# DeepLearnPhysics/u-resnet

Measured on AMD Instinct MI355X. Metric: fwd+bwd images/sec on 3D 192^3x1 U-ResNet, higher is better.
Workload: dtype f32; 1 GPU; cfg3_3d192_f8_b4; base_filters=8, num_class=3, batch_per_gpu=4, global_batch=4, step=zero_gradients+accum_gradients(fwd+loss+bwd)+allreduce+adam, parallelism=dp1

## Files before the change

### u-resnet_amd/csrc/conv_api.hip

```cpp
#include <dlfcn.h>
#include <stdarg.h>
#include <stdlib.h>
#include <stdio.h>
#include <string.h>

#include "bf16_common.h"

static thread_local char g_err[1024] = "";
void ursn_set_error(const char* fmt, ...) {
  va_list ap;
  va_start(ap, fmt);
  vsnprintf(g_err, sizeof(g_err), fmt, ap);
  va_end(ap);
}
extern "C" const char* ursn_last_error(void) { return g_err; }
static thread_local const char* g_kernel = "";
static long g_kernel_launches = 0;
void ursn_note_kernel(const char* name) { g_kernel = name; ++g_kernel_launches; }
void ursn_relabel_kernel(const char* name) { g_kernel = name; }
long ursn_kernel_launch_count() { return g_kernel_launches; }
extern "C" const char* ursn_last_kernel_name() { return g_kernel; }
extern "C" int ursn_abi_version(void) { return URSN_ABI_VERSION; }

namespace {
// ... 208 lines not shown
    if (g[i].ntaps == 0 && accumulate) continue;
    if (d.algo == 1) URSN_TRY(launch_gconv_naive(g[i], in, w, out, s));
    else URSN_TRY(launch_gconv_mfma(g[i], in, w, out, s));
  }
  return 0;
}

int tiled_conv_supported(const ursn_conv_desc& d, ConvPass pass);
int launch_tiled_conv(const ursn_conv_desc& d, ConvPass pass, const float* in, const float* w, float* out,
                      int accumulate, hipStream_t s);

static float* op_scratch_floats(size_t n) {
  static float* buf = nullptr;
  static size_t cap = 0;
  if (n > cap) {
    if (buf) (void)hipFree(buf);
    buf = nullptr; cap = 0;
    if (hipMalloc((void**)&buf, n * sizeof(float)) != hipSuccess) return nullptr;
    cap = n;
  }
  return buf;
}

int conv_dispatch(const ursn_conv_desc& d, ConvPass pass, const float* in, const float* w, float* out, int accumulate,
                  hipStream_t s) {
  if (d.vdz_z) {
    URSN_REQUIRE(pass == PASS_DGRAD && d.vdz_coef && d.vdz_out && tiled_conv_supported(d, pass), "conv: BatchNorm-backward apply on load (vdz_z) not supported for this shape / pass");
    return launch_tiled_conv(d, pass, in, w, out, accumulate, s);
  }
  if (d.bs_partial) {
    URSN_REQUIRE(pass == PASS_DGRAD && tiled_conv_supported(d, pass), "conv: fused BatchNorm-backward reductions (bs_partial) not supported for this shape / pass");
    return launch_tiled_conv(d, pass, in, w, out, accumulate, s);
  }
  if (d.in_mean && pass != PASS_DGRAD) {
    URSN_REQUIRE(d.in_rstd && d.in_beta && tiled_conv_supported(d, pass), "conv: normalise-on-load (in_mean) not supported for this shape / pass");
    return launch_tiled_conv(d, pass, in, w, out, accumulate, s);
  }
  if (d.pw_dy) {
    URSN_REQUIRE(pass == PASS_DGRAD, "conv: fused pointwise term (pw_dy) applies to the data gradient only");
    if (tiled_deconv_supported(d, pass))
      return launch_tiled_deconv(d, pass, in, w, out, accumulate, nullptr, 0.f, nullptr, nullptr, s);
    if (!d.in_split && igemm_conv_supported(d, pass))
      return launch_igemm_conv(d, pass, in, w, out, accumulate, nullptr, 0.f, nullptr, nullptr, s);
    URSN_REQUIRE(tiled_conv_supported(d, pass), "conv: fused pointwise term (pw_dy) not supported for this shape");
    return launch_tiled_conv(d, pass, in, w, out, accumulate, s);
  }
  if (d.in_split) {
    if (pointwise_conv_supported(d, pass, accumulate))
      return launch_pointwise_conv(d, pass, in, w, out, accumulate, nullptr, 0.f, nullptr, nullptr, s);
    URSN_REQUIRE(tiled_conv_supported(d, pass), "conv: split input (in_split=%d) not supported for this shape", d.in_split);
    return launch_tiled_conv(d, pass, in, w, out, accumulate, s);
  }
  if (d.algo == 3) {
    if (tiled_deconv_supported(d, pass))
// ... 215 lines not shown
    return launch_tiled_conv_bn(*d, x, w, y, (double*)scratch, eps, mean, rstd, s);
  }
  URSN_REQUIRE(reduce_scratch_bytes(V, d->cout, 2) <= scratch_bytes, "conv_forward_stats: scratch too small");
  URSN_TRY(conv_dispatch(*d, PASS_FWD, x, w, y, 0, s));
  return launch_bn_stats(y, ocs, V, d->cout, eps, mean, rstd, scratch, s);
}

extern "C" int ursn_conv_backward_data(const ursn_conv_desc* d, const float* dy, const float* w, float* dx,
                                       int32_t accumulate, void* stream) {
  URSN_REQUIRE(d && dy && w && dx, "conv_backward_data: null argument");
  if (d->dtype == 1) return bf16_conv_op(*d, PASS_DGRAD, dy, w, dx, accumulate, nullptr, 0, 0.f, nullptr, nullptr, (hipStream_t)stream);
  return conv_dispatch(*d, PASS_DGRAD, dy, w, dx, accumulate, (hipStream_t)stream);
}

int tiled_wgrad_supported(const ursn_conv_desc& d);
size_t tiled_wgrad_scratch_bytes(const ursn_conv_desc& d);
int valu_wgrad_supported(const ursn_conv_desc& d);
size_t valu_wgrad_scratch_bytes(const ursn_conv_desc& d);
int launch_valu_wgrad(const ursn_conv_desc& d, const float* x, const float* dy, float* dw, void* scratch, size_t scratch_bytes,
                      hipStream_t s);
int launch_tiled_wgrad(const ursn_conv_desc& d, const float* x, const float* dy, float* dw, void* scratch,
                       size_t scratch_bytes, hipStream_t s);

extern "C" int32_t ursn_conv_bs_blocks(const ursn_conv_desc* d) { return d ? tiled_conv_bs_blocks(*d) : 0; }

extern "C" int ursn_conv_plan(const ursn_conv_desc* d0, int32_t pass_, char* out, size_t cap) {
  URSN_REQUIRE(d0 && out && cap > 0 && pass_ >= 0 && pass_ <= 2, "conv_plan: bad argument");
  const ConvPass pass = (ConvPass)pass_;
  ursn_conv_desc d = *d0;
  const char* name = "gather";
  GatherGeom g[8];
  if (d.dtype == 1) {
    if (d.cin == 1) { d.cin = 8; d.in_cstride = 8; }
    const int n = build_geoms(d, pass, g);
    URSN_REQUIRE(n >= 1, "conv_plan: bad descriptor");
    int first = 0;
    while (first < n - 1 && g[first].ntaps == 0) ++first;
    if (pass == PASS_WGRAD) name = (d0->cin == 1 && b0wgrad_ok(g[0])) ? "b0wgrad" : b3wgrad_ok(g[0]) ? "b3wgrad" : bdwgrad_ok(g[0]) ? "bdwgrad" : bs2k8w_ok(g[0]) ? "bs2k8w" : (bwgrad_scratch_bytes(g[0]) ? "bwgrad" : "none");
    else if (d0->cin == 1 && pass == PASS_FWD && n == 1 && b0conv_ok(g[0])) name = "b0conv";
    else if (n == 1 && bs2k8_ok(g[0])) name = "bs2k8";
    else if (bdeconv_ok(g, n)) name = "bdeconv";
    else if (bsconv_ok(g, n)) name = "bsconv";
    else if (bpw_ok(g[first])) name = "bpw";
    else if (b3conv_ok(g[first])) name = "b3conv";
    else if (bcbconv_ok(g[first])) name = "bcbconv";
    else if (bdconv_ok(g[first])) name = "bdconv";
    else name = bconv_pack_elems(g[first]) ? "bconv" : "none";
    snprintf(out, cap, "%s", name);
    return 0;
  }
  URSN_REQUIRE(build_geoms(d, pass, g) >= 1, "conv_plan: bad descriptor");
  if (pass == PASS_WGRAD) {
    if (d.in_mean || (d.in_split && !pointwise_wgrad_supported(d))) name = tiled_wgrad_supported(d) ? "twgrad" : "none";
    else if (pointwise_wgrad_supported(d)) name = "pwgrad";
    else if (deep_wgrad_supported(d)) name = "dwgrad";
    else if (igemm_wgrad_supported(d)) name = "igemm_wgrad";
    else if (valu_wgrad_supported(d)) name = "vwgrad";
    else if (tiled_wgrad_supported(d)) name = "twgrad";
    else if (stride2_wgrad_supported(d)) name = "s2wgrad";
    else name = "wgrad_mfma";
  } else {
    if (d.vdz_z || d.bs_partial || (d.in_mean && pass != PASS_DGRAD)) name = tiled_conv_supported(d, pass) ? "tconv" : "none";
    else if (d.pw_dy && tiled_deconv_supported(d, pass)) name = "tdeconv+pw";
    else if (d.pw_dy) name = (!d.in_split && igemm_conv_supported(d, pass)) ? "igemm" : (tiled_conv_supported(d, pass) ? "tconv" : "none");
    else if (d.in_split) name = pointwise_conv_supported(d, pass, 0) ? "pconv" : (tiled_conv_supported(d, pass) ? "tconv" : "none");
    else if (pointwise_conv_supported(d, pass, 0)) name = "pconv";
    else if (deep_conv_supported(d, pass)) name = "dconv";
    else if (igemm_conv_supported(d, pass)) name = "igemm";
    else if (tiled_conv_supported(d, pass)) name = "tconv";
    else if (prefer_lds_scatter(d, pass)) name = "s2scatter";
    else if (tiled_deconv_supported(d, pass)) name = "tdeconv";
    else if (stride2_conv_supported(d, pass)) name = "s2conv";
    else name = "gconv_mfma";
  }
  snprintf(out, cap, "%s", name);
  return 0;
}

extern "C" size_t ursn_conv_wgrad_scratch_bytes(const ursn_conv_desc* d) {
  if (!d) return 0;
  GatherGeom g[8];
  if (d->dtype == 1) {
    ursn_conv_desc dd = *d;
    if (dd.cin == 1) { dd.cin = 8; dd.in_cstride = 8; }
    if (build_geoms(dd, PASS_WGRAD, g) != 1) return 0;
// ... 200 lines not shown
```

### u-resnet_amd/csrc/conv_igemm.hip

```cpp
#include <stdlib.h>

#include "conv_igemm_kernel.h"

bool ursn_igemm_on() {
  static const bool v = ursn_env_on("URSN_IGEMM");
  return v;
}

static bool make_igplan(const ursn_conv_desc& d, ConvPass pass, IGPlan& p, int& kcin, int& kcout) {
  if ((ursn_tiled_disabled() || !ursn_igemm_on()) && d.algo != 4) return false;
  if (d.transposed || d.k != 3 || d.stride != 1 || d.in_split || d.in_mean) return false;
  if (pass != PASS_FWD && pass != PASS_DGRAD) return false;
  p.flip = (pass == PASS_DGRAD);
  kcin = p.flip ? d.cout : d.cin;
  kcout = p.flip ? d.cin : d.cout;
  if ((kcin % 16) || (kcout % 16)) return false;
  if (kcin <= 16 && kcout <= 16 && d.algo != 4) return false;
  const int ics = d.in_cstride > 0 ? d.in_cstride : d.cin, ocs = d.out_cstride > 0 ? d.out_cstride : d.cout;
  if ((ics & 3) || (ocs & 3)) return false;
  p.mode = d.ndim;
  if (d.ndim == 3) { p.Z = d.in_sp[0]; p.Y = d.in_sp[1]; p.X = d.in_sp[2]; }
  else { p.Z = 1; p.Y = d.in_sp[0]; p.X = d.in_sp[1]; }
  static const int min_x = ursn_env_int("URSN_IGEMM_MINX", 5);
  if (p.X < min_x && d.algo != 4) return false;
  static const int at = ursn_env_int("URSN_IGEMM_ALLTAPS", 1);
  p.var = 0;
  if (at && p.mode == 3 && p.X <= 12) p.var = (p.X <= 6) ? 2 : 1;
  const bool at32 = at >= 1 && at != 16;
  if (!p.var && at32 && p.mode == 3 && (p.X % 16) != 0 && (p.X % 16) <= 8 && (p.X % 12) == 0) p.var = 1;
  if (p.X < 12 && !p.var && d.algo != 4) return false;
  const int BZ = p.mode == 3 ? (p.var == 2 ? 3 : 4) : 1, BY = p.mode == 3 ? (p.var == 2 ? 6 : 4) : 16,
            BX = p.var == 2 ? 6 : (p.var == 1 ? 12 : 16);
  p.nbz = (p.Z + BZ - 1) / BZ;
  p.nby = (p.Y + BY - 1) / BY;
  p.nbx = (p.X + BX - 1) / BX;
  p.gridx = d.n * p.nbz * p.nby * p.nbx;
  if (p.var == 2 || (p.var == 1 && !(at32 && kcout >= 32 && (int64_t)p.gridx * (kcout / 32) >= 384))) p.bm = 16;
  else if (p.var == 1) p.bm = 32;
  else if (kcout >= 64 && p.gridx >= 512) p.bm = 64;
  else if (kcout >= 32 && (int64_t)p.gridx * (kcout / 32) >= 384) p.bm = 32;
  else p.bm = 16;
  p.gridy = (kcout + p.bm - 1) / p.bm;
  const int HZ = p.mode == 3 ? BZ + 2 : 1, HY = BY + 2, HX = BX + 2;
  p.lds = ((size_t)4 * HZ * HY * HX * 4 + (size_t)2 * 16 * (p.bm + 16)) * sizeof(float);
  p.alltaps = (at && p.bm == 16) || (at >= 1 && at != 16 && p.bm == 32);
  if (d.pw_dy && !(p.flip && p.alltaps)) return false;
  if (p.alltaps) {
    {
      const int ics = d.in_cstride > 0 ? d.in_cstride : d.cin, ocs = d.out_cstride > 0 ? d.out_cstride : d.cout;
      if ((int64_t)p.Z * p.Y * p.X * (p.flip ? ocs : ics) * 4 >= (int64_t)0x80000000ll) return false;
    }
    const int kc = p.bm == 16 ? 16 : 8;
    p.lds = ((size_t)(kc / 4) * HZ * HY * HX * 4 + (size_t)(p.mode == 3 ? 27 : 9) * kc * p.bm) * sizeof(float);
    if (d.pw_dy) {
      const int nv = BZ * BY * BX;
      p.lds += ((size_t)(kc / 4) * nv * 4 + (size_t)p.bm * kc) * sizeof(float);
    }
    static const int pad_kb = ursn_env_int("URSN_IGEMM_LDS_KB", 0);
    if (pad_kb > 0 && p.lds < (size_t)pad_kb * 1024) p.lds = (size_t)pad_kb * 1024;
  }
  return true;
}

int igemm_conv_supported(const ursn_conv_desc& d, ConvPass pass) {
  IGPlan p;
  int a, b;
  return make_igplan(d, pass, p, a, b) ? 1 : 0;
}

size_t igemm_stats_scratch_doubles(const ursn_conv_desc& d) {
  IGPlan p;
  int a, b;
  if (!make_igplan(d, PASS_FWD, p, a, b)) return 0;
  return (size_t)p.gridx * p.gridy * 2 * p.bm;
}

template <int MODE, int BM>
static int dispatch_flags(const IGPlan& p, const IGemmArgs& a, hipStream_t s) {
  if (p.flip) return launch_ig<MODE, BM, true, false>(p, a, s);
  if (a.stats_partial) return launch_ig<MODE, BM, false, true>(p, a, s);
  return launch_ig<MODE, BM, false, false>(p, a, s);
}

template <int MODE>
static int dispatch_bm(const IGPlan& p, const IGemmArgs& a, hipStream_t s) {
  if (p.bm == 64) { ursn_note_kernel(p.flip ? "igemm_dgrad<64>" : "igemm<64>"); return dispatch_flags<MODE, 64>(p, a, s); }
  if (p.bm == 32 && p.alltaps) {
    ursn_note_kernel(p.flip ? "igemm_at_dgrad<32>" : "igemm_at<32>");
    if constexpr (MODE == 3) {
      if (p.var == 1) {
        if (p.flip) return launch_ig_at<3, 32, 8, true, false, 1>(p, a, s);
        if (a.stats_partial) return launch_ig_at<3, 32, 8, false, true, 1>(p, a, s);
        return launch_ig_at<3, 32, 8, false, false, 1>(p, a, s);
      }
    }
    if (p.flip) return launch_ig_at<MODE, 32, 8, true, false>(p, a, s);
    if (a.stats_partial) return launch_ig_at<MODE, 32, 8, false, true>(p, a, s);
    return launch_ig_at<MODE, 32, 8, false, false>(p, a, s);
  }
  if (p.bm == 32) { ursn_note_kernel(p.flip ? "igemm_dgrad<32>" : "igemm<32>"); return dispatch_flags<MODE, 32>(p, a, s); }
  if (p.alltaps) {
    ursn_note_kernel(p.flip ? "igemm_at_dgrad<16>" : "igemm_at<16>");
    if constexpr (MODE == 3) {
      if (p.var == 1) {
        if (p.flip) return launch_ig_at<3, 16, 16, true, false, 1>(p, a, s);
        if (a.stats_partial) return launch_ig_at<3, 16, 16, false, true, 1>(p, a, s);
        return launch_ig_at<3, 16, 16, false, false, 1>(p, a, s);
      }
      if (p.var == 2) {
        if (p.flip) return launch_ig_at<3, 16, 16, true, false, 2>(p, a, s);
        if (a.stats_partial) return launch_ig_at<3, 16, 16, false, true, 2>(p, a, s);
        return launch_ig_at<3, 16, 16, false, false, 2>(p, a, s);
      }
    }
    if (p.flip) return launch_ig_at<MODE, 16, 16, true, false>(p, a, s);
    if (a.stats_partial) return launch_ig_at<MODE, 16, 16, false, true>(p, a, s);
    return launch_ig_at<MODE, 16, 16, false, false>(p, a, s);
  }
  ursn_note_kernel(p.flip ? "igemm_dgrad<16>" : "igemm<16>");
  return dispatch_flags<MODE, 16>(p, a, s);
}

int launch_igemm_conv(const ursn_conv_desc& d, ConvPass pass, const float* in, const float* w, float* out,
                      int accumulate, double* stats_partial, float eps, float* mean, float* rstd, hipStream_t s) {
  IGPlan p;
  int kcin, kcout;
  URSN_REQUIRE(make_igplan(d, pass, p, kcin, kcout), "igemm conv: unsupported shape");
  const int ics = d.in_cstride > 0 ? d.in_cstride : d.cin, ocs = d.out_cstride > 0 ? d.out_cstride : d.cout;
  IGemmArgs a;
  a.in = in; a.w = w; a.out = out; a.stats_partial = stats_partial;
  a.N = d.n; a.Z = p.Z; a.Y = p.Y; a.X = p.X;
  a.cin = kcin; a.cout = kcout;
  a.in_cs = p.flip ? ocs : ics;
  a.out_cs = p.flip ? ics : ocs;
  a.cin_w = d.cin; a.cout_w = d.cout;
  a.nbz = p.nbz; a.nby = p.nby; a.nbx = p.nbx;
  a.accumulate = accumulate;
  a.pw_in = nullptr; a.pw_w = nullptr; a.pw_cs = 0; a.pw_ws = 0;
  if (d.pw_dy) {
    URSN_REQUIRE(p.flip && p.alltaps && d.pw_w, "igemm conv: fused pointwise term needs the all-taps data-gradient kernel");
    a.pw_in = d.pw_dy; a.pw_w = d.pw_w;
    a.pw_cs = d.pw_dy_cstride > 0 ? d.pw_dy_cstride : d.cout;
    a.pw_ws = d.cout;
    URSN_REQUIRE((a.pw_cs & 3) == 0, "igemm conv: pw_dy channel stride must be a multiple of 4");
  }
  URSN_TRY(p.mode == 3 ? dispatch_bm<3>(p, a, s) : dispatch_bm<2>(p, a, s));
  if (stats_partial) {
    const int64_t V = (int64_t)d.n * p.Z * p.Y * p.X;
    URSN_TRY(launch_bn_stats_final_blocked(stats_partial, p.gridx, kcout, p.bm, p.bm, (size_t)p.gridx * 2 * p.bm, V, eps, mean, rstd, s));
  }
  return 0;
}
```

### u-resnet_amd/csrc/conv_igemm_kernel.h

```cpp
#pragma once
#include <utility>

#include "ursn_common.h"
#include "buffer_stage.h"

typedef float ig_f32x4 __attribute__((ext_vector_type(4)));

template <int... Is, class F>
__device__ __forceinline__ void ig_static_for_impl(std::integer_sequence<int, Is...>, F&& f) {
  (f(std::integral_constant<int, Is>{}), ...);
}
template <int N, class F>
__device__ __forceinline__ void ig_static_for(F&& f) {
  ig_static_for_impl(std::make_integer_sequence<int, N>{}, static_cast<F&&>(f));
}

struct IGemmArgs {
  const float* in;
  const float* w;
  float* out;
  double* stats_partial;
  int N, Z, Y, X;
  int cin, cout;
  int in_cs, out_cs;
  int cin_w, cout_w;
  int nbz, nby, nbx;
  int accumulate;
  const float* pw_in;
  const float* pw_w;
  int pw_cs, pw_ws;
};

template <int MODE> struct IBox;
template <> struct IBox<3> { static constexpr int BZ = 4, BY = 4, BX = 16, NT = 27, KZ = 3; };
template <> struct IBox<2> { static constexpr int BZ = 1, BY = 16, BX = 16, NT = 9, KZ = 1; };
template <int MODE, int VAR> struct ABox : IBox<MODE> {};
template <> struct ABox<3, 1> { static constexpr int BZ = 4, BY = 4, BX = 12, NT = 27, KZ = 3; };
template <> struct ABox<3, 2> { static constexpr int BZ = 3, BY = 6, BX = 6, NT = 27, KZ = 3; };

template <int MODE, int BM, bool FLIP, bool STATS>
__global__ __launch_bounds__(256, 2) void igemm_conv_kernel(IGemmArgs a) {
  using B = IBox<MODE>;
  constexpr int BZ = B::BZ, BY = B::BY, BX = B::BX, NT = B::NT, KZ = B::KZ;
  constexpr int HZ = BZ + (KZ - 1), HY = BY + 2, HX = BX + 2, PS = HZ * HY * HX;
  constexpr int KC = 16, WS = BM + 16;
  constexpr int MT = BM / 16;
  constexpr int NH = (4 * PS + 255) / 256;
  extern __shared__ __attribute__((aligned(16))) float ilds[];
  float* hal = ilds;
  float* wl = ilds + 4 * PS * 4;

  const int tid = threadIdx.x, lane = tid & 63, wave = tid >> 6;
  const int il = lane & 15, kl = lane >> 4;
// ... 119 lines not shown
  }
  if constexpr (STATS) if (a.stats_partial) {
    __shared__ double red[4][2 * BM];
#pragma unroll
    for (int m = 0; m < MT; ++m)
#pragma unroll
      for (int r = 0; r < 4; ++r) {
        double u, w2;
        ursn_sacc_final(piv[m][r], s1[m][r], s2[m][r], nacc[m], u, w2);
#pragma unroll
        for (int o = 8; o >= 1; o >>= 1) { u += __shfl_xor(u, o); w2 += __shfl_xor(w2, o); }
        if (il == 0) {
          red[wave][16 * m + 4 * kl + r] = u;
          red[wave][BM + 16 * m + 4 * kl + r] = w2;
        }
      }
    __syncthreads();
    if (tid < 2 * BM)
      a.stats_partial[((size_t)blockIdx.y * gridDim.x + blockIdx.x) * 2 * BM + tid] =
          (red[0][tid] + red[1][tid]) + (red[2][tid] + red[3][tid]);
  }
}

template <int MODE, int BM, int KC, bool FLIP, bool STATS, int VAR = 0>
__global__ __launch_bounds__(256, 2) void igemm_at_kernel(IGemmArgs a) {
  using B = ABox<MODE, VAR>;
  constexpr int BZ = B::BZ, BY = B::BY, BX = B::BX, NT = B::NT, KZ = B::KZ;
  constexpr int NV = BZ * BY * BX, TPW = (NV + 63) / 64;
  constexpr int HZ = BZ + (KZ - 1), HY = BY + 2, HX = BX + 2, PS = HZ * HY * HX;
  constexpr int MT = BM / 16, NQ = KC / 4;
  constexpr int NH = (NQ * PS + 255) / 256;
  constexpr int NWF = NT * KC * BM / 4;
  constexpr int NW = (NWF + 255) / 256;
  extern __shared__ __attribute__((aligned(16))) float ilds[];
  float* hal = ilds;
  float* wl = ilds + NQ * PS * 4;

  const int tid = threadIdx.x, lane = tid & 63, wave = tid >> 6;
  const int il = lane & 15, kl = lane >> 4;
  int bid = ursn_xcd_block(blockIdx.x, gridDim.x);
  const int bx = bid % a.nbx; bid /= a.nbx;
  const int by = bid % a.nby; bid /= a.nby;
  const int bz = bid % a.nbz;
  const int n = bid / a.nbz;
  const int x0 = bx * BX, y0 = by * BY, z0 = bz * BZ;
  const int co0 = blockIdx.y * BM;

// ... 159 lines not shown
    if (pw) {
#pragma unroll
      for (int s = 0; s < NQ; ++s) {
        float av[MT], bv[TPW];
#pragma unroll
        for (int m = 0; m < MT; ++m) av[m] = pww[wb + ((size_t)m * KC + 4 * s) * 16];
#pragma unroll
        for (int v = 0; v < TPW; ++v) bv[v] = pwx[((size_t)s * NV + (vox[v] < 0 ? 0 : vox[v])) * 4 + kl];
#pragma unroll
        for (int v = 0; v < TPW; ++v)
#pragma unroll
          for (int m = 0; m < MT; ++m) acc[v][m] = __builtin_amdgcn_mfma_f32_16x16x4f32(av[m], bv[v], acc[v][m], 0, 0, 0);
      }
    }
  }

  float s1[MT][4], s2[MT][4], piv[MT][4], nacc[MT];
#pragma unroll
  for (int m = 0; m < MT; ++m) {
    nacc[m] = 0.f;
#pragma unroll
    for (int r = 0; r < 4; ++r) s1[m][r] = s2[m][r] = piv[m][r] = 0.f;
  }
#pragma unroll
  for (int v = 0; v < TPW; ++v) {
    if (vox[v] < 0) continue;
    const int lx = vox[v] % BX, r = vox[v] / BX;
    const int gx = x0 + lx, gy = y0 + r % BY, gz = z0 + r / BY;
    if (!(gz < a.Z && gy < a.Y && gx < a.X)) continue;
    float* op = a.out + ((((size_t)n * a.Z + gz) * a.Y + gy) * a.X + gx) * a.out_cs + co0;
#pragma unroll
    for (int m = 0; m < MT; ++m) {
      const int c = 16 * m + 4 * kl;
      if (co0 + c >= a.cout) continue;
      ig_f32x4 val = acc[v][m];
      if (a.accumulate) val += *(ig_f32x4*)(op + c);
      *(ig_f32x4*)(op + c) = val;
      if constexpr (STATS) {
#pragma unroll
        for (int r = 0; r < 4; ++r) {
          if (nacc[m] == 0.f) piv[m][r] = val[r];
          ursn_sacc(piv[m][r], s1[m][r], s2[m][r], val[r]);
        }
        nacc[m] += 1.f;
      }
    }
  }
  if constexpr (STATS) if (a.stats_partial) {
    __shared__ double red[4][2 * BM];
#pragma unroll
    for (int m = 0; m < MT; ++m)
#pragma unroll
      for (int r = 0; r < 4; ++r) {
        double u, w2;
        ursn_sacc_final(piv[m][r], s1[m][r], s2[m][r], nacc[m], u, w2);
#pragma unroll
        for (int o = 8; o >= 1; o >>= 1) { u += __shfl_xor(u, o); w2 += __shfl_xor(w2, o); }
        if (il == 0) {
          red[wave][16 * m + 4 * kl + r] = u;
          red[wave][BM + 16 * m + 4 * kl + r] = w2;
        }
      }
    __syncthreads();
    if (tid < 2 * BM)
      a.stats_partial[((size_t)blockIdx.y * gridDim.x + blockIdx.x) * 2 * BM + tid] =
          (red[0][tid] + red[1][tid]) + (red[2][tid] + red[3][tid]);
  }
}

struct IGPlan {
  bool alltaps;
  int var;
  int mode, bm;
  bool flip;
  int Z, Y, X, nbz, nby, nbx;
  size_t lds;
  int gridx, gridy;
};

template <int MODE, int BM, int KC, bool FLIP, bool STATS, int VAR = 0>
static int launch_ig_at(const IGPlan& p, const IGemmArgs& a, hipStream_t s) {
  auto kern = igemm_at_kernel<MODE, BM, KC, FLIP, STATS, VAR>;
  static size_t attr_lds = 48 * 1024;
  if (p.lds > attr_lds) {
    URSN_HIP(hipFuncSetAttribute((const void*)kern, hipFuncAttributeMaxDynamicSharedMemorySize, (int)p.lds));
    attr_lds = p.lds;
  }
  hipLaunchKernelGGL(kern, dim3(p.gridx, p.gridy), dim3(256), p.lds, s, a);
  URSN_HIP(hipGetLastError());
  return 0;
}

template <int MODE, int BM, bool FLIP, bool STATS>
static int launch_ig(const IGPlan& p, const IGemmArgs& a, hipStream_t s) {
  auto kern = igemm_conv_kernel<MODE, BM, FLIP, STATS>;
  static size_t attr_lds = 48 * 1024;
  if (p.lds > attr_lds) {
    URSN_HIP(hipFuncSetAttribute((const void*)kern, hipFuncAttributeMaxDynamicSharedMemorySize, (int)p.lds));
    attr_lds = p.lds;
  }
  hipLaunchKernelGGL(kern, dim3(p.gridx, p.gridy), dim3(256), p.lds, s, a);
  URSN_HIP(hipGetLastError());
  return 0;
}
```

### u-resnet_amd/csrc/net.hip

```cpp
#include <math.h>
#include <stdio.h>
#include <stdlib.h>
#include <string.h>

#include <map>
#include <string>
#include <vector>

#include "ursn_common.h"
#include "net_bf16.h"

int conv_dispatch(const ursn_conv_desc& d, ConvPass pass, const float* in, const float* w, float* out, int accumulate,
                  hipStream_t s);
int wgrad_dispatch(const ursn_conv_desc& d, const float* x, const float* dy, float* dw, void* scratch,
                   size_t scratch_bytes, hipStream_t s);

namespace {

struct Act {
  float* p = nullptr;
  float* g = nullptr;
  int C = 0, cs = 0, lvl = 0;
  int flag = -1;
};

struct Layer {
  std::string name;
  int kind = 0;
  int k = 3, stride = 1, cin = 0, cout = 0, lin = 0, lout = 0;
  int relu = 0;
  int64_t w_off = 0, b_off = 0, w_n = 0;
  ursn_conv_desc desc;
  float *z = nullptr, *dz = nullptr, *mean = nullptr, *rstd = nullptr;
  float* coef = nullptr;
  int zcs = 0;
};

struct Unit {
  std::string scope;
  int sc = -1, c1 = -1, c2 = -1;
// ... 284 lines not shown
      }
    }
  }
  n->red_scratch = A.take(red + 256);
  n->dc_scratch = dcf ? A.floats((int64_t)dcf + 64) : nullptr;
  {
    size_t red2 = 0;
    for (const Unit& u : n->units) {
      if (u.sc < 0) continue;
      const Layer& L = n->layers[u.sc];
      size_t r = reduce_scratch_bytes((int64_t)c.max_batch * n->lvox[L.lout], L.cout, 3);
      if (r > red2) red2 = r;
      for (int nb = 1; nb <= c.max_batch; ++nb) {
        ursn_conv_desc d = L.desc;
        d.n = nb;
        r = pointwise_stats_scratch_doubles(d) * sizeof(double);
        if (r > red2) red2 = r;
      }
    }
    n->red_scratch2 = A.take(red2 + 256);
  }
  n->wg_scratch_bytes = wg;
  n->wg_scratch = tr ? A.take(wg + 256) : nullptr;
  n->bs_scratch = tr ? (double*)A.take((size_t)16384 * 3 * 8 * sizeof(double)) : nullptr;

  n->sizes.n_params = poff;
  n->sizes.n_layers = (int64_t)n->layers.size();
  n->sizes.n_tensors = 2 * (int64_t)n->layers.size();
  n->sizes.workspace_bytes = (int64_t)((A.off + 255) & ~(size_t)255);
  return 0;
}

extern "C" const char* ursn_last_kernel_name();
hipEvent_t prof_event(ursn_net* n) {
  if (n->ev_used == n->ev_pool.size()) {
    hipEvent_t e;
    if (hipEventCreate(&e) != hipSuccess) return nullptr;
    n->ev_pool.push_back(e);
  }
  return n->ev_pool[n->ev_used++];
}
struct ProfScope {
  ursn_net* n; hipStream_t s; int idx = -1; bool range = false;
  ProfScope(ursn_net* n_, hipStream_t s_, int layer, int pass, double flops, double bytes) : n(n_), s(s_) {
    if (ursn_roctx_on()) { ursn_roctx_push(n->layers[layer].name.c_str(), pass); range = true; }
    if (!n->profile || n->prof.size() > 200000) return;
    ursn_net::ProfRec r{layer, pass, "", flops, bytes, prof_event(n), prof_event(n), ursn_kernel_launch_count(), 1};
    if (!r.e0 || !r.e1) return;
    hipEventRecord(r.e0, s);
    n->prof.push_back(r);
    idx = (int)n->prof.size() - 1;
  }
  ~ProfScope() { if (range) ursn_roctx_pop(); }
  void done(const char* kernel) {
    if (idx < 0) return;
    n->prof[idx].kernel = kernel;
    long nl = ursn_kernel_launch_count() - n->prof[idx].l0;
    n->prof[idx].launches = nl > 0 ? (int)nl : 1;
    hipEventRecord(n->prof[idx].e1, s);
  }
};
double layer_macs(const ursn_net* n, const Layer& L, int N) {
  double taps = 1;
  for (int j = 0; j < n->cfg.ndim; ++j) taps *= L.k;
  double vox = (double)N * (L.kind ? n->lvox[L.lin] : n->lvox[L.lout]);
  return vox * taps * L.cin * L.cout;
}
double layer_bytes(const ursn_net* n, const Layer& L, int N) {
  return 4.0 * ((double)N * n->lvox[L.lin] * L.cin + (double)N * n->lvox[L.lout] * L.cout + (double)L.w_n);
}

int conv_stats(ursn_net* n, int li, const Act& in, int N, hipStream_t s, const Act* in2 = nullptr, int aff = -1,
               void* red_scratch = nullptr) {
  if (!red_scratch) red_scratch = n->red_scratch;
  Layer& L = n->layers[li];
  ursn_conv_desc d = L.desc;
  d.n = N;
  d.in_cstride = in.cs;
  d.out_cstride = L.zcs;
  if (in2) { d.in_split = in.C; d.in2_cstride = in2->cs; d.x2 = in2->p; }
  if (aff >= 0) {
// ... 253 lines not shown
    URSN_TRY(wgrad_dispatch(d, in.p, L.dz, n->grads + L.w_off, n->wg_scratch, n->wg_scratch_bytes, ws));
    ps.done(ursn_last_kernel_name());
  }
  if (dgrad_done_elsewhere) {
    ProfScope pd(n, s, li, 1, 2.0 * layer_macs(n, L, N), layer_bytes(n, L, N));
    pd.done("(fused into conv1 dgrad)");
  }
  if (need_dgrad) {
    bool acc = take_flag(n, in);
    if (in2) URSN_REQUIRE(take_flag(n, *in2) == acc, "split input: the two halves disagree on gradient initialisation");
    d = bwd_desc(n, li, in, N, in2, fused_sc);
    n->bs_layer = -1;
    static const bool bs_off = !ursn_env_on("URSN_FUSE_BN_BWD_REDUCE");
    if (bs && bs->li >= 0 && !bs_off) {
      const Layer& T = n->layers[bs->li];
      ursn_conv_desc t = d;
      t.bs_z = T.z; t.bs_z_cstride = T.zcs; t.bs_mean = T.mean; t.bs_rstd = T.rstd; t.bs_beta = n->params + T.b_off;
      t.bs_relu = bs->relu; t.bs_mask = bs->mask;
      if (bs->li2 >= 0) {
        const Layer& T2 = n->layers[bs->li2];
        t.bs_z2 = T2.z; t.bs_z2_cstride = T2.zcs; t.bs_mean2 = T2.mean; t.bs_rstd2 = T2.rstd;
      }
      t.bs_partial = n->bs_scratch;
      const bool fits = T.cout == 8 && T.zcs == 8 && in.C == 8 && in.cs == 8 && !in2 &&
                        (bs->li2 < 0 || n->layers[bs->li2].zcs == 8) && (bs->relu != 2 || bs->mask);
      const int blocks = fits ? tiled_conv_bs_blocks(t) : 0;
      if (blocks > 0 && blocks <= 16384) { d = t; n->bs_layer = bs->li; n->bs_blocks = blocks; }
    }
    ProfScope pd(n, s, li, 1, 2.0 * layer_macs(n, L, N), layer_bytes(n, L, N));
    if (n->dc_scratch && deep_conv_supported(d, PASS_DGRAD))
      URSN_TRY(launch_deep_conv(d, PASS_DGRAD, L.dz, n->params + L.w_off, in.g, acc ? 1 : 0, n->dc_scratch, nullptr, 0.f, nullptr, nullptr, s));
    else
      URSN_TRY(conv_dispatch(d, PASS_DGRAD, L.dz, n->params + L.w_off, in.g, acc ? 1 : 0, s));
    pd.done(ursn_last_kernel_name());
  }
  return 0;
}

bool vdz_ok(ursn_net* n, int li, const Act& in, int N, bool two_z_target) {
  static const bool on = ursn_env_on("URSN_FUSE_BN_BWD_APPLY");
  const bool off = !on || two_z_target;
  const Layer& L = n->layers[li];
  if (off || n->cfg.ndim != 3 || L.kind || L.k != 3 || L.stride != 1 || L.cin != 8 || L.cout != 8 || L.zcs != 8 || in.C != 8 || in.cs != 8 || !in.g)
    return false;
  ursn_conv_desc d = L.desc;
  d.n = N; d.in_cstride = in.cs; d.out_cstride = L.zcs;
  d.vdz_z = L.z; d.vdz_coef = L.coef; d.vdz_out = L.dz;
  return tiled_conv_supported(d, PASS_DGRAD) != 0;
}

// ... 3 lines not shown
  Layer& L = n->layers[li];
  BnBwdArgs a;
  memset(&a, 0, sizeof(a));
  a.dy = dy; a.dycs = dycs; a.y = mask ? nullptr : y; a.ycs = ycs; a.mask = mask;
  a.z = L.z; a.zcs = L.zcs; a.mean = L.mean; a.rstd = L.rstd; a.dz = L.dz; a.dzcs = L.zcs;
  a.dbeta = n->grads + L.b_off;
  a.beta = n->params + L.b_off;
  if (li2 >= 0) {
    Layer& L2 = n->layers[li2];
    a.z2 = L2.z; a.z2cs = L2.zcs; a.mean2 = L2.mean; a.rstd2 = L2.rstd; a.dz2 = L2.dz; a.dz2cs = L2.zcs;
    a.dbeta2 = n->grads + L2.b_off;
  }
  a.dres = dres; a.drescs = drescs; a.dres_accumulate = dres_acc;
  a.V = (int64_t)N * n->lvox[L.lout]; a.C = L.cout; a.relu = relu; a.scratch = n->red_scratch;
  if (L.zcs != L.cout && li2 < 0 && !relu && dycs == L.zcs && !dres) { a.C = L.zcs; a.Cw = L.cout; }
  if (n->bs_layer == li && a.C == n->bs_C) { a.pre_partial = n->bs_scratch; a.pre_nblocks = n->bs_blocks; }
  n->bs_layer = -1;
  n->bs_C = 8;
  n->vdz_layer = -1;
  if (fuse_in && li2 < 0 && !dres && !mask && !y && dycs == L.zcs && vdz_ok(n, li, *fuse_in, N, fuse_two_z)) {
    a.coef_out = L.coef;
    n->vdz_layer = li; n->vdz_relu = relu; n->vdz_g = dy; n->vdz_cs = dycs;
  }
  ProfScope ps(n, s, li, 5, 0.0, 4.0 * a.V * a.C * (2.0 * (2 + (relu && !mask) + (li2 >= 0)) + 1 + (li2 >= 0) + (dres != nullptr)));
  URSN_TRY(launch_bn_bwd(a, s));
  ps.done("bn_bwd");
  return 0;
}

int unit_bwd(ursn_net* n, Unit& u, int N, hipStream_t s, const BsTarget* in_target = nullptr) {
  if (u.sc >= 0) {
    URSN_TRY(bn_back(n, u.c2, u.out.g, u.out.cs, u.out.p, u.out.cs, 1, u.sc, nullptr, 0, 0, N, s, u.jmask));
  } else {
    bool acc = take_flag(n, u.in);
    URSN_TRY(bn_back(n, u.c2, u.out.g, u.out.cs, u.out.p, u.out.cs, 1, -1, u.in.g, u.in.cs, acc ? 1 : 0, N, s, u.jmask));
  }
  BsTarget t1;
  t1.li = u.c1;
  if (u.a1_virtual) {
    Act z1 = u.a1;
    z1.p = n->layers[u.c1].z; z1.cs = n->layers[u.c1].zcs;
    URSN_TRY(conv_bwd(n, u.c2, z1, true, N, s, nullptr, -1, false, u.c1, &t1));
  } else {
    URSN_TRY(conv_bwd(n, u.c2, u.a1, true, N, s, nullptr, -1, false, -1, &t1));
  }
  URSN_TRY(bn_back(n, u.c1, u.a1.g, u.a1.cs, nullptr, 0, 0, -1, nullptr, 0, 0, N, s, nullptr, (u.in2.C || u.sc >= 0) ? nullptr : &u.in,
                   in_target && in_target->li2 >= 0));
  const Act* in2 = u.in2.C ? &u.in2 : nullptr;
  bool fuse = false;
// ... 512 lines not shown
```

### u-resnet_amd/csrc/ursn_common.h

```cpp
#pragma once
#include <hip/hip_runtime.h>
#include <stdint.h>
#include <stddef.h>
#include <stdlib.h>

#include "../../include/uresnet_hip.h"

void ursn_set_error(const char* fmt, ...);
void ursn_note_kernel(const char* name);
void ursn_relabel_kernel(const char* name);
#ifdef __HIPCC__
#ifndef URSN_XCD_REMAP
#define URSN_XCD_REMAP 1
#endif
__device__ __forceinline__ int ursn_xcd_block(int b, int G) {
#if URSN_XCD_REMAP
  const int q = G >> 3, r = G & 7, x = b & 7, i = b >> 3;
  return (x < r ? x * (q + 1) : r * (q + 1) + (x - r) * q) + i;
#else
  return b;
#endif
}

__device__ __forceinline__ void ursn_sacc(float piv, float& s1, float& s2, float v) {
// ... 93 lines not shown
enum ConvPass { PASS_FWD = 0, PASS_DGRAD = 1, PASS_WGRAD = 2 };
int build_geoms(const ursn_conv_desc& d, ConvPass pass, GatherGeom* out8);

struct BnStats {
  double* sum;
  float* mean;
  float* rstd;
};

size_t reduce_scratch_bytes(int64_t voxels, int channels, int nsums);
int reduce_nblocks(int64_t voxels, int channels);

int launch_bn_stats(const float* z, int zcs, int64_t V, int C, float eps, float* mean, float* rstd,
                    void* scratch, hipStream_t s);
int launch_bn_stats_final(const double* partial, int nblocks, int C, int PC, int64_t V, float eps, float* mean,
                          float* rstd, hipStream_t s);
int launch_bn_stats_final_blocked(const double* partial, int nblocks, int C, int CB, int PC, size_t blk_stride, int64_t V, float eps,
                                  float* mean, float* rstd, hipStream_t s);
int tiled_conv_supported(const ursn_conv_desc& d, ConvPass pass);
size_t tiled_conv_stats_scratch_doubles(const ursn_conv_desc& d);
int launch_tiled_conv_bn(const ursn_conv_desc& d, const float* in, const float* w, float* out, double* scratch,
                         float eps, float* mean, float* rstd, hipStream_t s);
int tiled_wgrad_supported(const ursn_conv_desc& d);
int tiled_conv_bs_blocks(const ursn_conv_desc& d);
int igemm_conv_supported(const ursn_conv_desc& d, ConvPass pass);
size_t igemm_stats_scratch_doubles(const ursn_conv_desc& d);
int launch_igemm_conv(const ursn_conv_desc& d, ConvPass pass, const float* in, const float* w, float* out,
                      int accumulate, double* stats_partial, float eps, float* mean, float* rstd, hipStream_t s);
int igemm_wgrad_supported(const ursn_conv_desc& d);
size_t igemm_wgrad_scratch_bytes(const ursn_conv_desc& d);
int launch_igemm_wgrad(const ursn_conv_desc& d, const float* x, const float* dy, float* dw, void* scratch,
                       size_t scratch_bytes, hipStream_t s);
int deep_conv_supported(const ursn_conv_desc& d, ConvPass pass);
size_t deep_conv_scratch_floats(const ursn_conv_desc& d, ConvPass pass);
size_t deep_conv_stats_scratch_doubles(const ursn_conv_desc& d);
int launch_deep_conv(const ursn_conv_desc& d, ConvPass pass, const float* in, const float* w, float* out, int accumulate,
                     float* scratch, double* stats_partial, float eps, float* mean, float* rstd, hipStream_t s);
int deep_wgrad_supported(const ursn_conv_desc& d);
size_t deep_wgrad_scratch_bytes(const ursn_conv_desc& d);
int launch_deep_wgrad(const ursn_conv_desc& d, const float* x, const float* dy, float* dw, void* scratch, size_t scratch_bytes,
                      hipStream_t s);
int pointwise_conv_supported(const ursn_conv_desc& d, ConvPass pass, int accumulate);
size_t pointwise_stats_scratch_doubles(const ursn_conv_desc& d);
int launch_pointwise_conv(const ursn_conv_desc& d, ConvPass pass, const float* in, const float* w, float* out,
                          int accumulate, double* stats_partial, float eps, float* mean, float* rstd, hipStream_t s);
int pointwise_wgrad_supported(const ursn_conv_desc& d);
size_t pointwise_wgrad_scratch_bytes(const ursn_conv_desc& d);
int launch_pointwise_wgrad(const ursn_conv_desc& d, const float* x, const float* dy, float* dw, void* scratch,
                           size_t scratch_bytes, hipStream_t s);
// ... 79 lines not shown
```

Before: 67.71 images/s.

## Fuse BatchNorm-backward reductions into igemm dgrad epilogue for wider channels

Extends the fused BatchNorm-backward partial reductions (sum of g and g·xhat, optionally a second branch) from the tiled conv to the implicit-GEMM data-gradient kernel. This lets 16- and 32-channel layers, not only 8-channel ones, fuse the reductions into the conv epilogue. The aim is to drop a separate BN-backward reduction pass over the activations. In exchange the igemm epilogue gets more registers (double accumulators, prefetched z/mask values) and gains template variants, which may lower occupancy.

```diff
diff --git a/u-resnet_amd/csrc/conv_api.hip b/u-resnet_amd/csrc/conv_api.hip
--- a/u-resnet_amd/csrc/conv_api.hip
+++ b/u-resnet_amd/csrc/conv_api.hip
@@ -254,6 +254,22 @@
   return buf;
 }
 
+static int bs_route(const ursn_conv_desc& d) {
+  ursn_conv_desc plain = d;
+  plain.bs_partial = nullptr;
+  const bool ig_plain = !d.in_split && (d.algo == 0 || d.algo == 4) && igemm_conv_supported(plain, PASS_DGRAD);
+  if (!d.pw_dy && d.algo == 0 && deep_conv_supported(plain, PASS_DGRAD)) return 0;
+  if (ig_plain) return igemm_conv_supported(d, PASS_DGRAD) ? 2 : 0;
+  return tiled_conv_supported(d, PASS_DGRAD) ? 1 : 0;
+}
+
+int conv_bs_blocks(const ursn_conv_desc& d) {
+  ursn_conv_desc t = d;
+  t.bs_partial = (double*)1;
+  const int r = bs_route(t);
+  return r == 2 ? igemm_conv_bs_blocks(t) : (r == 1 ? tiled_conv_bs_blocks(t) : 0);
+}
+
 int conv_dispatch(const ursn_conv_desc& d, ConvPass pass, const float* in, const float* w, float* out, int accumulate,
                   hipStream_t s) {
   if (d.vdz_z) {
@@ -261,7 +277,8 @@
     return launch_tiled_conv(d, pass, in, w, out, accumulate, s);
   }
   if (d.bs_partial) {
-    URSN_REQUIRE(pass == PASS_DGRAD && tiled_conv_supported(d, pass), "conv: fused BatchNorm-backward reductions (bs_partial) not supported for this shape / pass");
+    URSN_REQUIRE(pass == PASS_DGRAD && bs_route(d) != 0, "conv: fused BatchNorm-backward reductions (bs_partial) not supported for this shape / pass");
+    if (bs_route(d) == 2) return launch_igemm_conv(d, pass, in, w, out, accumulate, nullptr, 0.f, nullptr, nullptr, s);
     return launch_tiled_conv(d, pass, in, w, out, accumulate, s);
   }
   if (d.in_mean && pass != PASS_DGRAD) {
@@ -523,7 +540,7 @@
 int launch_tiled_wgrad(const ursn_conv_desc& d, const float* x, const float* dy, float* dw, void* scratch,
                        size_t scratch_bytes, hipStream_t s);
 
-extern "C" int32_t ursn_conv_bs_blocks(const ursn_conv_desc* d) { return d ? tiled_conv_bs_blocks(*d) : 0; }
+extern "C" int32_t ursn_conv_bs_blocks(const ursn_conv_desc* d) { return d ? conv_bs_blocks(*d) : 0; }
 
 extern "C" int ursn_conv_plan(const ursn_conv_desc* d0, int32_t pass_, char* out, size_t cap) {
   URSN_REQUIRE(d0 && out && cap > 0 && pass_ >= 0 && pass_ <= 2, "conv_plan: bad argument");
@@ -561,7 +578,8 @@
     else if (stride2_wgrad_supported(d)) name = "s2wgrad";
     else name = "wgrad_mfma";
   } else {
-    if (d.vdz_z || d.bs_partial || (d.in_mean && pass != PASS_DGRAD)) name = tiled_conv_supported(d, pass) ? "tconv" : "none";
+    if (d.bs_partial && !d.vdz_z) name = pass != PASS_DGRAD ? "none" : (bs_route(d) == 2 ? "igemm" : (bs_route(d) == 1 ? "tconv" : "none"));
+    else if (d.vdz_z || (d.in_mean && pass != PASS_DGRAD)) name = tiled_conv_supported(d, pass) ? "tconv" : "none";
     else if (d.pw_dy && tiled_deconv_supported(d, pass)) name = "tdeconv+pw";
     else if (d.pw_dy) name = (!d.in_split && igemm_conv_supported(d, pass)) ? "igemm" : (tiled_conv_supported(d, pass) ? "tconv" : "none");
     else if (d.in_split) name = pointwise_conv_supported(d, pass, 0) ? "pconv" : (tiled_conv_supported(d, pass) ? "tconv" : "none");
diff --git a/u-resnet_amd/csrc/conv_igemm.hip b/u-resnet_amd/csrc/conv_igemm.hip
--- a/u-resnet_amd/csrc/conv_igemm.hip
+++ b/u-resnet_amd/csrc/conv_igemm.hip
@@ -45,6 +45,11 @@
   p.lds = ((size_t)4 * HZ * HY * HX * 4 + (size_t)2 * 16 * (p.bm + 16)) * sizeof(float);
   p.alltaps = (at && p.bm == 16) || (at >= 1 && at != 16 && p.bm == 32);
   if (d.pw_dy && !(p.flip && p.alltaps)) return false;
+  if (d.bs_partial) {
+    const int zcs = d.bs_z_cstride > 0 ? d.bs_z_cstride : kcout, z2cs = d.bs_z2_cstride > 0 ? d.bs_z2_cstride : kcout;
+    if (!(p.flip && p.alltaps && p.mode == 3) || (zcs & 3) || (d.bs_z2 && (z2cs & 3))) return false;
+    if (d.bs_z2 && p.bm == 32 && p.var == 1) return false;
+  }
   if (p.alltaps) {
     {
       const int ics = d.in_cstride > 0 ? d.in_cstride : d.cin, ocs = d.out_cstride > 0 ? d.out_cstride : d.cout;
@@ -68,6 +73,14 @@
   return make_igplan(d, pass, p, a, b) ? 1 : 0;
 }
 
+int igemm_conv_bs_blocks(const ursn_conv_desc& d) {
+  ursn_conv_desc t = d;
+  t.bs_partial = (double*)1;
+  IGPlan p;
+  int a, b;
+  return make_igplan(t, PASS_DGRAD, p, a, b) ? p.gridx : 0;
+}
+
 size_t igemm_stats_scratch_doubles(const ursn_conv_desc& d) {
   IGPlan p;
   int a, b;
@@ -89,10 +102,14 @@
     ursn_note_kernel(p.flip ? "igemm_at_dgrad<32>" : "igemm_at<32>");
     if constexpr (MODE == 3) {
       if (p.var == 1) {
+        if (p.flip && a.bs_partial) return a.bs_z2 ? launch_ig_at<3, 32, 8, true, false, 1, 2>(p, a, s) : launch_ig_at<3, 32, 8, true, false, 1, 1>(p, a, s);
         if (p.flip) return launch_ig_at<3, 32, 8, true, false, 1>(p, a, s);
         if (a.stats_partial) return launch_ig_at<3, 32, 8, false, true, 1>(p, a, s);
         return launch_ig_at<3, 32, 8, false, false, 1>(p, a, s);
       }
+    }
+    if constexpr (MODE == 3) {
+      if (p.flip && a.bs_partial) return a.bs_z2 ? launch_ig_at<3, 32, 8, true, false, 0, 2>(p, a, s) : launch_ig_at<3, 32, 8, true, false, 0, 1>(p, a, s);
     }
     if (p.flip) return launch_ig_at<MODE, 32, 8, true, false>(p, a, s);
     if (a.stats_partial) return launch_ig_at<MODE, 32, 8, false, true>(p, a, s);
@@ -103,15 +120,20 @@
     ursn_note_kernel(p.flip ? "igemm_at_dgrad<16>" : "igemm_at<16>");
     if constexpr (MODE == 3) {
       if (p.var == 1) {
+        if (p.flip && a.bs_partial) return a.bs_z2 ? launch_ig_at<3, 16, 16, true, false, 1, 2>(p, a, s) : launch_ig_at<3, 16, 16, true, false, 1, 1>(p, a, s);
         if (p.flip) return launch_ig_at<3, 16, 16, true, false, 1>(p, a, s);
         if (a.stats_partial) return launch_ig_at<3, 16, 16, false, true, 1>(p, a, s);
         return launch_ig_at<3, 16, 16, false, false, 1>(p, a, s);
       }
       if (p.var == 2) {
+        if (p.flip && a.bs_partial) return a.bs_z2 ? launch_ig_at<3, 16, 16, true, false, 2, 2>(p, a, s) : launch_ig_at<3, 16, 16, true, false, 2, 1>(p, a, s);
         if (p.flip) return launch_ig_at<3, 16, 16, true, false, 2>(p, a, s);
         if (a.stats_partial) return launch_ig_at<3, 16, 16, false, true, 2>(p, a, s);
         return launch_ig_at<3, 16, 16, false, false, 2>(p, a, s);
       }
+    }
+    if constexpr (MODE == 3) {
+      if (p.flip && a.bs_partial) return a.bs_z2 ? launch_ig_at<3, 16, 16, true, false, 0, 2>(p, a, s) : launch_ig_at<3, 16, 16, true, false, 0, 1>(p, a, s);
     }
     if (p.flip) return launch_ig_at<MODE, 16, 16, true, false>(p, a, s);
     if (a.stats_partial) return launch_ig_at<MODE, 16, 16, false, true>(p, a, s);
@@ -144,7 +166,21 @@
     a.pw_ws = d.cout;
     URSN_REQUIRE((a.pw_cs & 3) == 0, "igemm conv: pw_dy channel stride must be a multiple of 4");
   }
+  a.bs_z = a.bs_mean = a.bs_rstd = a.bs_beta = a.bs_z2 = a.bs_mean2 = a.bs_rstd2 = nullptr;
+  a.bs_mask = nullptr; a.bs_partial = nullptr; a.bs_z_cs = a.bs_z2_cs = 0; a.bs_relu = 0; a.bs_C = kcout;
+  if (d.bs_partial) {
+    URSN_REQUIRE(p.flip && p.alltaps && p.mode == 3 && d.bs_z && d.bs_mean && d.bs_rstd && (d.bs_relu != 1 || d.bs_beta) &&
+                 (d.bs_relu != 2 || d.bs_mask) && (!d.bs_z2 || (d.bs_mean2 && d.bs_rstd2)),
+                 "igemm conv: incomplete fused BatchNorm-backward arguments");
+    a.bs_partial = d.bs_partial; a.bs_z = d.bs_z; a.bs_mean = d.bs_mean; a.bs_rstd = d.bs_rstd; a.bs_beta = d.bs_beta;
+    a.bs_z2 = d.bs_z2; a.bs_mean2 = d.bs_mean2; a.bs_rstd2 = d.bs_rstd2; a.bs_mask = (const unsigned long long*)d.bs_mask;
+    a.bs_z_cs = d.bs_z_cstride > 0 ? d.bs_z_cstride : kcout; a.bs_z2_cs = d.bs_z2_cstride > 0 ? d.bs_z2_cstride : kcout;
+    a.bs_relu = d.bs_relu;
+  }
   URSN_TRY(p.mode == 3 ? dispatch_bm<3>(p, a, s) : dispatch_bm<2>(p, a, s));
+  if (d.bs_partial)
+    ursn_relabel_kernel(p.bm == 32 ? (d.bs_z2 ? "igemm_at_dgrad<32>+bnred2" : "igemm_at_dgrad<32>+bnred")
+                                   : (d.bs_z2 ? "igemm_at_dgrad<16>+bnred2" : "igemm_at_dgrad<16>+bnred"));
   if (stats_partial) {
     const int64_t V = (int64_t)d.n * p.Z * p.Y * p.X;
     URSN_TRY(launch_bn_stats_final_blocked(stats_partial, p.gridx, kcout, p.bm, p.bm, (size_t)p.gridx * 2 * p.bm, V, eps, mean, rstd, s));
diff --git a/u-resnet_amd/csrc/conv_igemm_kernel.h b/u-resnet_amd/csrc/conv_igemm_kernel.h
--- a/u-resnet_amd/csrc/conv_igemm_kernel.h
+++ b/u-resnet_amd/csrc/conv_igemm_kernel.h
@@ -29,6 +29,11 @@
   const float* pw_in;
   const float* pw_w;
   int pw_cs, pw_ws;
+  const float* bs_z;  const float* bs_mean;  const float* bs_rstd;  const float* bs_beta;
+  const float* bs_z2; const float* bs_mean2; const float* bs_rstd2;
+  const unsigned long long* bs_mask;
+  double* bs_partial;
+  int bs_z_cs, bs_z2_cs, bs_relu, bs_C;
 };
 
 template <int MODE> struct IBox;
@@ -194,7 +199,7 @@
   }
 }
 
-template <int MODE, int BM, int KC, bool FLIP, bool STATS, int VAR = 0>
+template <int MODE, int BM, int KC, bool FLIP, bool STATS, int VAR = 0, int BS = 0>
 __global__ __launch_bounds__(256, 2) void igemm_at_kernel(IGemmArgs a) {
   using B = ABox<MODE, VAR>;
   constexpr int BZ = B::BZ, BY = B::BY, BX = B::BX, NT = B::NT, KZ = B::KZ;
@@ -400,6 +405,41 @@
 #pragma unroll
     for (int r = 0; r < 4; ++r) s1[m][r] = s2[m][r] = piv[m][r] = 0.f;
   }
+  constexpr int BT = BS ? TPW : 1, BMT = BS ? MT : 1;
+  ig_f32x4 bzv[BT][BMT], bzv2[BS == 2 ? BT : 1][BMT], bold[BT][BMT];
+  unsigned bmw[BT][BMT][4];
+  double bg[BMT][4], bgx[BMT][4], bgx2[BS == 2 ? BMT : 1][4];
+  if constexpr (BS != 0) {
+#pragma unroll
+    for (int m = 0; m < MT; ++m)
+#pragma unroll
+      for (int r = 0; r < 4; ++r) {
+        bg[m][r] = bgx[m][r] = 0.0;
+        if constexpr (BS == 2) bgx2[m][r] = 0.0;
+      }
+#pragma unroll
+    for (int v = 0; v < TPW; ++v) {
+      if (vox[v] < 0) continue;
+      const int lx = vox[v] % BX, r = vox[v] / BX;
+      const int gx = x0 + lx, gy = y0 + r % BY, gz = z0 + r / BY;
+      if (!(gz < a.Z && gy < a.Y && gx < a.X)) continue;
+      const size_t gv = (((size_t)n * a.Z + gz) * a.Y + gy) * a.X + gx;
+#pragma unroll
+      for (int m = 0; m < MT; ++m) {
+        const int c = co0 + 16 * m + 4 * kl;
+        if (c >= a.cout) continue;
+        bzv[v][m] = *(const ig_f32x4*)(a.bs_z + gv * a.bs_z_cs + c);
+        if constexpr (BS == 2) bzv2[v][m] = *(const ig_f32x4*)(a.bs_z2 + gv * a.bs_z2_cs + c);
+        if (a.accumulate) bold[v][m] = *(const ig_f32x4*)(a.out + gv * a.out_cs + c);
+        if (a.bs_relu == 2) {
+          const size_t e = gv * (size_t)a.bs_C + c;
+          const unsigned* mw = (const unsigned*)(a.bs_mask + (e >> 8) * 4) + (((unsigned)e & 255u) >> 7);
+#pragma unroll
+          for (int j = 0; j < 4; ++j) bmw[v][m][j] = mw[2 * j];
+        }
+      }
+    }
+  }
 #pragma unroll
   for (int v = 0; v < TPW; ++v) {
     if (vox[v] < 0) continue;
@@ -412,8 +452,40 @@
       const int c = 16 * m + 4 * kl;
       if (co0 + c >= a.cout) continue;
       ig_f32x4 val = acc[v][m];
-      if (a.accumulate) val += *(ig_f32x4*)(op + c);
+      if constexpr (BS != 0) {
+        if (a.accumulate) val += bold[v][m];
+      } else {
+        if (a.accumulate) val += *(ig_f32x4*)(op + c);
+      }
       *(ig_f32x4*)(op + c) = val;
+      if constexpr (BS != 0) {
+        const ig_f32x4 zv = bzv[v][m];
+        const ig_f32x4 mu = *(const ig_f32x4*)(a.bs_mean + co0 + c), rs = *(const ig_f32x4*)(a.bs_rstd + co0 + c);
+        ig_f32x4 g = val;
+        if (a.bs_relu == 1) {
+          const ig_f32x4 be = *(const ig_f32x4*)(a.bs_beta + co0 + c);
+#pragma unroll
+          for (int j = 0; j < 4; ++j)
+            if (!(__builtin_fmaf(zv[j], rs[j], be[j] - mu[j] * rs[j]) > 0.f)) g[j] = 0.f;
+        } else if (a.bs_relu == 2) {
+          const size_t gv = (((size_t)n * a.Z + gz) * a.Y + gy) * a.X + gx;
+          const unsigned bit = ((unsigned)(gv * (size_t)a.bs_C + co0 + c) & 127u) >> 2;
+#pragma unroll
+          for (int j = 0; j < 4; ++j)
+            if (!((bmw[v][m][j] >> bit) & 1u)) g[j] = 0.f;
+        }
+#pragma unroll
+        for (int j = 0; j < 4; ++j) {
+          const double gd = (double)g[j];
+          bg[m][j] += gd;
+          bgx[m][j] += gd * (double)((zv[j] - mu[j]) * rs[j]);
+        }
+        if constexpr (BS == 2) {
+          const ig_f32x4 mu2 = *(const ig_f32x4*)(a.bs_mean2 + co0 + c), rs2 = *(const ig_f32x4*)(a.bs_rstd2 + co0 + c);
+#pragma unroll
+          for (int j = 0; j < 4; ++j) bgx2[m][j] += (double)g[j] * (double)((bzv2[v][m][j] - mu2[j]) * rs2[j]);
+        }
+      }
       if constexpr (STATS) {
 #pragma unroll
         for (int r = 0; r < 4; ++r) {
@@ -443,6 +515,31 @@
     if (tid < 2 * BM)
       a.stats_partial[((size_t)blockIdx.y * gridDim.x + blockIdx.x) * 2 * BM + tid] =
           (red[0][tid] + red[1][tid]) + (red[2][tid] + red[3][tid]);
+  }
+  if constexpr (BS != 0) {
+    __shared__ double bred[4][3 * BM];
+#pragma unroll
+    for (int m = 0; m < MT; ++m)
+#pragma unroll
+      for (int r = 0; r < 4; ++r) {
+        double u = bg[m][r], w2 = bgx[m][r], x2 = 0.0;
+        if constexpr (BS == 2) x2 = bgx2[m][r];
+#pragma unroll
+        for (int o = 8; o >= 1; o >>= 1) {
+          u += __shfl_xor(u, o);
+          w2 += __shfl_xor(w2, o);
+          if constexpr (BS == 2) x2 += __shfl_xor(x2, o);
+        }
+        if (il == 0) {
+          bred[wave][16 * m + 4 * kl + r] = u;
+          bred[wave][BM + 16 * m + 4 * kl + r] = w2;
+          bred[wave][2 * BM + 16 * m + 4 * kl + r] = x2;
+        }
+      }
+    __syncthreads();
+    if (tid < 3 * BM && co0 + tid % BM < a.cout)
+      a.bs_partial[((size_t)blockIdx.x * 3 + tid / BM) * a.bs_C + co0 + tid % BM] =
+          (bred[0][tid] + bred[1][tid]) + (bred[2][tid] + bred[3][tid]);
   }
 }
 
@@ -456,9 +553,9 @@
   int gridx, gridy;
 };
 
-template <int MODE, int BM, int KC, bool FLIP, bool STATS, int VAR = 0>
+template <int MODE, int BM, int KC, bool FLIP, bool STATS, int VAR = 0, int BS = 0>
 static int launch_ig_at(const IGPlan& p, const IGemmArgs& a, hipStream_t s) {
-  auto kern = igemm_at_kernel<MODE, BM, KC, FLIP, STATS, VAR>;
+  auto kern = igemm_at_kernel<MODE, BM, KC, FLIP, STATS, VAR, BS>;
   static size_t attr_lds = 48 * 1024;
   if (p.lds > attr_lds) {
     URSN_HIP(hipFuncSetAttribute((const void*)kern, hipFuncAttributeMaxDynamicSharedMemorySize, (int)p.lds));
diff --git a/u-resnet_amd/csrc/net.hip b/u-resnet_amd/csrc/net.hip
--- a/u-resnet_amd/csrc/net.hip
+++ b/u-resnet_amd/csrc/net.hip
@@ -16,6 +16,8 @@
                    size_t scratch_bytes, hipStream_t s);
 
 namespace {
+
+constexpr size_t BS_SCRATCH_DOUBLES = (size_t)16384 * 3 * 8;
 
 struct Act {
   float* p = nullptr;
@@ -346,7 +348,7 @@
   }
   n->wg_scratch_bytes = wg;
   n->wg_scratch = tr ? A.take(wg + 256) : nullptr;
-  n->bs_scratch = tr ? (double*)A.take((size_t)16384 * 3 * 8 * sizeof(double)) : nullptr;
+  n->bs_scratch = tr ? (double*)A.take(BS_SCRATCH_DOUBLES * sizeof(double)) : nullptr;
 
   n->sizes.n_params = poff;
   n->sizes.n_layers = (int64_t)n->layers.size();
@@ -376,11 +378,11 @@
     idx = (int)n->prof.size() - 1;
   }
   ~ProfScope() { if (range) ursn_roctx_pop(); }
-  void done(const char* kernel) {
+  void done(const char* kernel, int launches = 0) {
     if (idx < 0) return;
     n->prof[idx].kernel = kernel;
     long nl = ursn_kernel_launch_count() - n->prof[idx].l0;
-    n->prof[idx].launches = nl > 0 ? (int)nl : 1;
+    n->prof[idx].launches = launches > 0 ? launches : (nl > 0 ? (int)nl : 1);
     hipEventRecord(n->prof[idx].e1, s);
   }
 };
@@ -680,10 +682,12 @@
         t.bs_z2 = T2.z; t.bs_z2_cstride = T2.zcs; t.bs_mean2 = T2.mean; t.bs_rstd2 = T2.rstd;
       }
       t.bs_partial = n->bs_scratch;
-      const bool fits = T.cout == 8 && T.zcs == 8 && in.C == 8 && in.cs == 8 && !in2 &&
-                        (bs->li2 < 0 || n->layers[bs->li2].zcs == 8) && (bs->relu != 2 || bs->mask);
-      const int blocks = fits ? tiled_conv_bs_blocks(t) : 0;
-      if (blocks > 0 && blocks <= 16384) { d = t; n->bs_layer = bs->li; n->bs_blocks = blocks; }
+      const int tC = T.cout;
+      const bool fits = (tC == 8 || tC == 16 || tC == 32) && T.zcs == tC && in.C == tC && in.cs == tC && !in2 &&
+                        (bs->li2 < 0 || n->layers[bs->li2].zcs == tC) && (bs->relu != 2 || bs->mask) &&
+                        !(n->dc_scratch && deep_conv_supported(d, PASS_DGRAD));
+      const int blocks = fits ? conv_bs_blocks(t) : 0;
+      if (blocks > 0 && (size_t)blocks * 3 * tC <= BS_SCRATCH_DOUBLES) { d = t; n->bs_layer = bs->li; n->bs_blocks = blocks; n->bs_C = tC; }
     }
     ProfScope pd(n, s, li, 1, 2.0 * layer_macs(n, L, N), layer_bytes(n, L, N));
     if (n->dc_scratch && deep_conv_supported(d, PASS_DGRAD))
@@ -733,9 +737,11 @@
     a.coef_out = L.coef;
     n->vdz_layer = li; n->vdz_relu = relu; n->vdz_g = dy; n->vdz_cs = dycs;
   }
-  ProfScope ps(n, s, li, 5, 0.0, 4.0 * a.V * a.C * (2.0 * (2 + (relu && !mask) + (li2 >= 0)) + 1 + (li2 >= 0) + (dres != nullptr)));
+  const int passes = (a.pre_partial ? 0 : 1) + (a.coef_out ? 0 : 1);
+  ProfScope ps(n, s, li, 5, 0.0, 4.0 * a.V * a.C * ((double)passes * (2 + (relu && !mask) + (li2 >= 0)) +
+                                                    (a.coef_out ? 0 : 1 + (li2 >= 0) + (dres != nullptr))));
   URSN_TRY(launch_bn_bwd(a, s));
-  ps.done("bn_bwd");
+  ps.done("bn_bwd", passes + 1);
   return 0;
 }
 
diff --git a/u-resnet_amd/csrc/ursn_common.h b/u-resnet_amd/csrc/ursn_common.h
--- a/u-resnet_amd/csrc/ursn_common.h
+++ b/u-resnet_amd/csrc/ursn_common.h
@@ -139,9 +139,11 @@
 int launch_tiled_conv_bn(const ursn_conv_desc& d, const float* in, const float* w, float* out, double* scratch,
                          float eps, float* mean, float* rstd, hipStream_t s);
 int tiled_wgrad_supported(const ursn_conv_desc& d);
+int conv_bs_blocks(const ursn_conv_desc& d);
 int tiled_conv_bs_blocks(const ursn_conv_desc& d);
 int igemm_conv_supported(const ursn_conv_desc& d, ConvPass pass);
 size_t igemm_stats_scratch_doubles(const ursn_conv_desc& d);
+int igemm_conv_bs_blocks(const ursn_conv_desc& d);
 int launch_igemm_conv(const ursn_conv_desc& d, ConvPass pass, const float* in, const float* w, float* out,
                       int accumulate, double* stats_partial, float eps, float* mean, float* rstd, hipStream_t s);
 int igemm_wgrad_supported(const ursn_conv_desc& d);
```

After: 67.62 images/s. Within noise of the previous version (-0.1%).
